# HKUST-Aerial-Robotics/ESVO

Hardware: AMD Instinct MI355X
Metric: mapped events/sec (stereo TS raster + block matching + LM depth refinement + fusion), events resident in HBM before the timed region; exactly K ticks between two synchronisations, i.e. including the fill and the drain of the two-deep tick pipeline (`sustained`: the same workload over 1600 ticks) (higher is better)
Workload: dtype f64

## Files before the change

esvo_amd/csrc/api_core.hip:

```cpp
#include "context.hpp"

namespace esvo_host {
thread_local std::string g_create_error;
}

namespace {

void invert3x3(const double* P, double* Kinv, double* Kinv_t) {
  const double a = P[0], b = P[1], cc = P[2], d = P[4], e = P[5], f = P[6], g = P[8], hh = P[9], i = P[10];
  const double det = a * (e * i - f * hh) - b * (d * i - f * g) + cc * (d * hh - e * g);
  const double id = 1.0 / det;
  Kinv[0] = (e * i - f * hh) * id; Kinv[1] = (cc * hh - b * i) * id; Kinv[2] = (b * f - cc * e) * id;
  Kinv[3] = (f * g - d * i) * id;  Kinv[4] = (a * i - cc * g) * id;  Kinv[5] = (cc * d - a * f) * id;
  Kinv[6] = (d * hh - e * g) * id; Kinv[7] = (b * g - a * hh) * id;  Kinv[8] = (a * e - b * d) * id;
  for (int r = 0; r < 3; ++r) Kinv_t[r] = (Kinv[r * 3 + 0] * P[3] + Kinv[r * 3 + 1] * P[7]) + Kinv[r * 3 + 2] * P[11];
}

int validate_params(const esvo_params_t* p, std::string& why) {
  if (p->ls_norm != ESVO_LSNORM_TDIST && p->ls_norm != ESVO_LSNORM_L2) { why = "LSnorm must be Tdist or l2 (DepthProblemSolver.cpp:121-131 exits on anything else)"; return ESVO_ERR_UNSUPPORTED; }
  if (p->bm_step < 1) { why = "BM_step must be >= 1"; return ESVO_ERR_INVALID_ARG; }
  if (p->patch_size_x < 1 || p->patch_size_x > 64 || p->patch_size_y < 1 || p->patch_size_y > 40) { why = "patch size must be within 1..64 x 1..40"; return ESVO_ERR_UNSUPPORTED; }
  if (p->median_blur_kernel_size < 0 || p->median_blur_kernel_size > 3) { why = "median_blur_kernel_size must be 0..3 (kernel 2k + 1)"; return ESVO_ERR_UNSUPPORTED; }
  if (p->max_event_queue_len < 0 || p->max_event_queue_len > TSQ_LMAX) { why = "max_event_queue_len must be 0 (one stamp per pixel) or 1..32"; return ESVO_ERR_UNSUPPORTED; }
  if (p->bm_max_disparity < p->bm_min_disparity || p->bm_min_disparity < 0) { why = "bad disparity range"; return ESVO_ERR_INVALID_ARG; }
// ... 133 lines not shown
  CK(h->d_tick_ev.alloc(E));
  CK(h->d_match_slots.alloc(E));
  CK(h->d_match_flags.alloc(E)); CK(h->d_match_prefix.alloc(E));
  for (int k = 0; k < 2; ++k) CK(h->front[k].d_matches.alloc(E));
  if (E >= LM_SPLIT_MIN_EVENTS) {
    CK(h->d_lm_fvec0.alloc(E * 7 * 16)); CK(h->d_lm_fnorm0.alloc(E));
    CK(h->d_lm_meta.alloc(E)); CK(h->d_lm_order.alloc(E));
    CK(h->d_lm_hist.alloc(2 * 32 * 64));
    CK(hipMemset(h->d_lm_hist, 0, sizeof(u32) * 2 * 32 * 64));
  }
  if (E > LM_TWO_QUEUES_MAX_EVENTS) {
    for (int k = 0; k < 2; ++k) { CK(h->front[k].d_lm_pix_order.alloc(E)); CK(h->d_lm_sort_rows[k].alloc(E)); }
    CK(h->d_lm_sort_hist.alloc(voxel_hist_words(E)));
  }
  if (h->bm_dedupe_on && E >= h->bm_dedupe_min) CK(h->d_bm_dedupe.alloc(npx + 4 + 2 * E));
  CK(h->d_clk.alloc(2 * clk_words(h->max_ev)));
  CK(hipMemset(h->d_clk, 0, sizeof(u64) * 2 * clk_words(h->max_ev)));
  int khz = 0;
  if (hipDeviceGetAttribute(&khz, hipDeviceAttributeWallClockRate, h->device) != hipSuccess || khz <= 0) khz = 100000;
  h->stats.clk_ref_khz = (uint32_t)khz;
  for (int k = 0; k < 2; ++k) {
    CK(h->front[k].d_pt_slots.alloc(E));
    CK(h->front[k].d_pt_flags.alloc(E)); CK(h->front[k].d_pt_prefix.alloc(E));
    CK(h->front[k].d_scan_tmp_l.alloc(scan_scratch_elems(std::max(E, npx)) + 8));
  }
  CK(h->d_pts_tmp.alloc(E));
  for (int k = 0; k < 2; ++k) CK(h->front[k].d_stage.alloc(E));
  for (int k = 0; k < 2; ++k) CK(h->front[k].d_counters.alloc(CNT_ROW));
  for (int k = 0; k < 2; ++k) CK(hipMemset(h->front[k].d_counters, 0, sizeof(u32) * CNT_ROW));
  CK(h->h_counters.alloc(CNT_ROW * 2));
  std::memset(h->h_counters, 0, sizeof(u32) * CNT_ROW * 2);
  CK(h->h_pin.alloc(2 * ((size_t)h->max_poses * 17 + 16)));
  CK(h->d_scan_tmp.alloc(scan_scratch_elems(std::max(E, npx)) + 8)); CK(h->d_scan_tmp_b.alloc(scan_scratch_elems(std::max(E, npx)) + 8));
  CK(h->d_cnt_b.alloc(CNTB_ROW)); CK(hipMemset(h->d_cnt_b, 0, sizeof(u32) * CNTB_ROW));
  CK(h->h_cnt_b.alloc(CNTB_ROW * CNTB_ROWS));
  std::memset(h->h_cnt_b, 0, sizeof(u32) * CNTB_ROW * CNTB_ROWS);
  for (int k = 0; k < 2; ++k) { h->front[k].d_clk = h->d_clk + (size_t)k * clk_words(h->max_ev); h->front[k].h_counters = h->h_counters + CNT_ROW * k; h->back[k].h_cnt = h->h_cnt_b + CNTB_ROW * k; }
  CK(h->d_halo_viol.alloc(2));
  return ESVO_OK;
}

int alloc_window_and_map(esvo_context* h) {
  const size_t npx = (size_t)h->W * h->H, E = h->max_ev;
  h->win_cap = (u32)std::max<int64_t>((int64_t)h->prm.max_window_points, (int64_t)E) + 2 * (u32)E;
  CK(h->d_win.alloc(h->win_cap));
  h->max_frames = (u32)std::max(h->prm.max_fusion_frames + 2, 512);
  if (h->prm.fusion_strategy == ESVO_FUSION_CONST_POINTS)
    h->max_frames = std::max(h->max_frames, (u32)(1.5 * h->prm.max_fusion_points) + 4u);
  h->slot_used.assign(h->max_frames + 1, 0);
  h->n_pose_slots = std::min<u32>(h->max_frames + 1, h->n_pose_slots);
  CK(h->d_frame_pose_T.alloc((size_t)h->n_pose_slots * h->max_poses * 16));
  CK(h->d_fr_table.alloc(2 * (3 * (size_t)h->max_frames + 1))); CK(h->h_fr_table.alloc(2 * (3 * (size_t)h->max_frames + 1)));
  for (int k = 0; k < 2; ++k) { h->back[k].d_fr_table = h->d_fr_table + k * (h->d_fr_table.cap() / 2); h->back[k].h_fr_table = h->h_fr_table + k * (h->h_fr_table.cap() / 2); }
  CK(h->d_prop.alloc(h->win_cap));
  const size_t n_tiles = fuse_front_tiles(h);
  CK(h->d_tile_pts.alloc(n_tiles * h->fuse_tile_cap)); CK(h->d_over_pts.alloc(h->win_cap));
  CK(h->d_tile_count.alloc(n_tiles));
  CK(h->d_cell_count.alloc(npx)); CK(h->d_cell_offset.alloc(npx));
  h->fuse_slice_cap = (u32)((n_tiles + 63) / 64) * FUSE_TILE * FUSE_TILE;
  CK(h->d_cell_list.alloc((size_t)16 * 64 * h->fuse_slice_cap));
  CK(h->d_fuse_ctr.alloc(2112 + 64));
  CK(hipMemset(h->d_fuse_ctr + 2112, 0, sizeof(u32) * 64));
  CK(h->d_rec_ids.alloc(n_tiles * h->fuse_tile_rec + (size_t)h->win_cap * 9));
  for (int k = 0; k < 2; ++k) CK(h->d_map_mem[k].alloc(map_buffer_bytes(npx)));
  h->d_map = reinterpret_cast<MapCell*>(h->d_map_mem[0].get()); h->d_map2 = reinterpret_cast<MapCell*>(h->d_map_mem[1].get());
  CK(h->d_owner_max.alloc(npx)); CK(h->d_owner_min.alloc(npx));
  CK(h->d_own_w.alloc(E)); CK(h->d_lkeep.alloc(E));
  h->codes_bytes = (E + 7) / 8 * 8;
  CK(h->d_codes.alloc(h->codes_bytes));
  CK(h->d_sel.alloc(E));
  CK(h->d_evmap.alloc(npx + 64));
  CK(h->d_reg_ab.alloc(npx)); CK(h->d_reg_cd.alloc(npx));
  CK(h->d_exp_flags.alloc(npx)); CK(h->d_exp_prefix.alloc(npx));
  CK(h->d_export.alloc(npx)); CK(h->d_export_cell.alloc(npx));
  return ESVO_OK;
}

int create_events_and_pools(esvo_context* h) {
  for (int k = 0; k < 2; ++k) CK(h->ts_ev[k].create());
  CK(h->ev_frame.create());
  for (int k = 0; k < 2; ++k) CK(h->front[k].own_ev.create());
  for (int k = 0; k < 2; ++k) { CK(h->back[k].ev.create()); CK(h->pose[k].released.create()); }
  if (h->tl_on) { CK(h->tl_ref.create()); CK(hipEventRecord(h->tl_ref, h->stream)); CK(hipEventSynchronize(h->tl_ref)); }
  CK(h->evt_trk_read.create(hipEventDisableTiming));
  for (int cam = 0; cam < 2; ++cam) CK(h->evt_ingest[cam].create(hipEventDisableTiming));
  CK(h->h_pose_pool.alloc(16 * (size_t)h->max_poses * esvo_context::POSE_POOL));
  for (int i = 0; i < esvo_context::POSE_POOL; ++i) CK(h->pool_evt[i].create());
  for (int i = 0; i < 16; ++i) h->T_world_obs[i] = h->T_world_frame[i] = (i % 5 == 0) ? 1.0 : 0.0;
  return ESVO_OK;
}
#undef CK

}

namespace esvo_host {

void fill_dev_params(esvo_context* h) {
  const esvo_params_t& p = h->prm;
  DevParams& d = h->dp;
  d.W = h->W; d.H = h->H;
  d.wx = p.patch_size_x; d.wy = p.patch_size_y;
  d.dmin = p.bm_min_disparity; d.dmax = p.bm_max_disparity; d.step = p.bm_step; d.updown = p.bm_updown ? 1 : 0;
  d.zncc_thr = p.bm_zncc_threshold;
  d.baseline_f = h->baseline * d.camL.P[0];
  d.td_nu = p.td_nu; d.td_scale = p.td_scale; d.td_scale2 = p.td_scale * p.td_scale;
  const double td_stdvar = std::sqrt(p.td_nu / (p.td_nu - 2) * (p.td_scale * p.td_scale));
  d.td_stdvar2 = td_stdvar * td_stdvar;
// ... 302 lines not shown
```

esvo_amd/csrc/api_window.hip:

```cpp
#include "context.hpp"

namespace esvo_host {

static int read_counters_b(esvo_context* h, int row, bool sync) {
  HIPCHK(hipMemcpyAsync(h->h_cnt_b + CNTB_ROW * row, h->d_cnt_b, sizeof(u32) * CNTB_ROW, hipMemcpyDeviceToHost, h->stream_b));
  if (sync) HIPCHK(hipStreamSynchronize(h->stream_b));
  return ESVO_OK;
}
int back_after_front(esvo_context* h) {
  HIPCHK(hipEventRecord(h->ev_frame, h->stream));
  HIPCHK(hipStreamWaitEvent(h->stream_b, h->ev_frame, 0));
  return ESVO_OK;
}
void collect_back(esvo_context* h, int par) {
  if (!h->back_pending[par]) return;
  h->back_pending[par] = false;
  const BackSlot& B = h->back[par];
  esvo_stats_t& s = h->stats;
  s.last_fusions = B.h_cnt[CNTB_FUSIONS];
  if (h->routed && h->h_cnt_b[CNTB_ROW * CNTB_ROW_HALO + par]) {
    s.halo_violations = h->h_cnt_b[CNTB_ROW * CNTB_ROW_HALO + par];
    h->halo_error = true;
  }
  if (h->prm.regularization) s.last_map_size = B.h_cnt[CNTB_REG_ELEMS];
// ... 126 lines not shown
      HIPCHK(hipEventRecord(h->pool_evt[ps], h->stream_b));
    } else if (h->pro.active) {
      h->pro.b_src = h->pose[pose_buf].d_T; h->pro.b_dst = dst; h->pro.b_bytes = sizeof(double) * 16 * m;
      h->pro.ev_b = h->pose[pose_buf].released;
    } else {
      HIPCHK(hipMemcpyAsync(dst, h->pose[pose_buf].d_T, sizeof(double) * 16 * m, hipMemcpyDeviceToDevice, h->stream_b));
      HIPCHK(hipEventRecord(h->pose[pose_buf].released, h->stream_b));
    }
  }
  h->frames.push_back(FrameRec{off, count, slot, 1});
  h->n_window_frames++;
  if (apply_policy) apply_window_policy(h);
  return ESVO_OK;
}

int run_fuse(esvo_context* h, int par, const double* T_world_obs, bool naive) {
  BackSlot& B = h->back[par];
  u32* host = B.h_fr_table;
  u32 nf = 0;
  for (size_t q = h->frames.size(); q-- > 0;)
    if (h->frames[q].count) ++nf;
  if (nf > h->max_frames) { (void)flush_deferred_copies(h); FAIL(ESVO_ERR_CAPACITY, "too many non-empty frames in the fusion window"); }
  u32* cum = host;
  u32* off = host + (nf + 1);
  u32* slot = off + nf;
  u32 total = 0, i = 0;
  for (size_t q = h->frames.size(); q-- > 0;) {
    const FrameRec& f = h->frames[q];
    if (f.count == 0) continue;
    cum[i] = total; off[i] = f.off; slot[i] = f.slot;
    total += f.count;
    ++i;
  }
  cum[nf] = total;
  hipStream_t sb = h->stream_b;
  hipEvent_t tail_ev[2] = {nullptr, nullptr};
  u32* dtab = B.d_fr_table;
  if (h->pro.active) {
    const esvo_context::DeferredCopies d = h->pro;
    h->pro = esvo_context::DeferredCopies();
    launch_back_prologue(host, dtab, sizeof(u32) * (3 * (size_t)nf + 1), d.a_src, d.a_dst, d.a_bytes, d.b_src, d.b_dst, d.b_bytes, sb,
                         d.a_flags, d.a_prefix, d.a_slots);
    tail_ev[0] = d.ev_a; tail_ev[1] = d.ev_b;
  } else {
    launch_upload_words(host, dtab, sizeof(u32) * (3 * (size_t)nf + 1), sb);
  }
  std::memcpy(h->T_world_frame, T_world_obs, sizeof(double) * 16);
  FuseArgs a;
  a.win = h->d_win;
  a.fr_cum = dtab; a.fr_off = dtab + (nf + 1); a.fr_slot = a.fr_off + nf;
  a.n_frames = nf; a.n_pts = total;
  a.frame_pose_T = h->d_frame_pose_T; a.max_poses = h->max_poses;
  rigid_inverse(h->T_world_frame, a.T_frame_world);
  a.prop = h->d_prop;
  a.tile_count = h->d_tile_count; a.tile_pts = h->d_tile_pts; a.tile_cap = h->fuse_tile_cap;
  a.over_pts = h->d_over_pts; a.over_count = h->d_fuse_ctr + FUSE_CTR_OVER_COUNT;
  a.rec_ids = h->d_rec_ids; a.tile_rec = h->fuse_tile_rec; a.rec_cursor = h->d_fuse_ctr + FUSE_CTR_REC_CURSOR;
  a.cell_count = h->d_cell_count; a.cell_offset = h->d_cell_offset; a.cell_list = h->d_cell_list; a.slice_cap = h->fuse_slice_cap;
  a.class_count = h->d_fuse_ctr; a.class_total = h->d_fuse_ctr + FUSE_CTR_CLASS_TOTAL;
  a.lds_cap = h->fuse_lds_cap; a.pmax_plus1 = h->fuse_pmax_plus1; a.d_total = h->d_cnt_b + CNTB_RECORDS;
  a.map = h->d_map; a.d_num_fusion = h->d_cnt_b + CNTB_FUSIONS;
  a.n_touched = h->d_cnt_b + CNTB_TOUCHED;
  a.naive = naive ? 1 : 0;
  a.owner_max = h->prm.regularization ? h->d_owner_max : nullptr;
  a.owner_min = h->d_owner_min; a.n_reg_elems = h->prm.regularization ? h->d_cnt_b + CNTB_REG_ELEMS : nullptr;
  if (total > h->win_cap) {
    for (hipEvent_t e : tail_ev) if (e) hipEventRecord(e, sb);
    FAIL(ESVO_ERR_CAPACITY, "window points exceed capacity");
  }
  const bool timed = h->stage_events_on;
  B.timed = timed;
  if (timed) hipEventRecord(B.ev.e[BE_FU0], sb);
  launch_fuse(a, h->dp, sb);
  if (timed) hipEventRecord(B.ev.e[BE_FU1], sb);
  h->d_map_cur = h->d_map;
  h->map_id_bound = total * ((naive || h->dp.fusion_radius == 0) ? 4u : 9u);
  const bool do_clean = naive ? false : (h->prm.clean_requires_full_window ? (h->n_window_frames >= (size_t)h->prm.max_fusion_frames) : true);
  if (do_clean) launch_clean(h->d_map, h->dp, sb);
  if (timed) hipEventRecord(B.ev.e[BE_CL1], sb);
  if (h->prm.regularization && !naive) {
    launch_reg_view(h->d_map, h->d_map2, h->d_owner_max, h->d_owner_min, h->d_reg_ab, h->d_reg_cd, h->d_cnt_b + CNTB_REG_ELEMS, h->dp, sb);
    const u64 band_cells = (u64)std::max(h->dp.band_y1 - h->dp.band_y0, 1) * (u64)h->W;
    const bool sparse = h->reg_sparse_forced >= 0 ? h->reg_sparse_forced == 1 : (u64)h->stats.last_map_size * 10u < band_cells;
    launch_reg_apply(h->d_map, h->d_map2, h->d_owner_max, h->d_owner_min, h->d_reg_ab, h->d_reg_cd, h->d_cnt_b + CNTB_REG_ELEMS, h->dp, sb, sparse);
    h->d_map_cur = h->d_map2;
  }
  HIPCHK(hipMemcpyAsync(B.h_cnt, h->d_cnt_b, sizeof(u32) * CNTB_ROW, hipMemcpyDeviceToHost, sb));
  if (h->routed) HIPCHK(hipMemcpyAsync(h->h_cnt_b + CNTB_ROW * CNTB_ROW_HALO + par, h->d_halo_viol, sizeof(u32), hipMemcpyDeviceToHost, sb));
  hipEventRecord(B.ev.e[BE_RG1], sb);
  for (hipEvent_t e : tail_ev) if (e) hipEventRecord(e, sb);
  HIPCHK(hipGetLastError());
  h->back_pending[par] = true;
  return ESVO_OK;
}

int export_map(esvo_context* h, std::vector<esvo_depth_point_t>& out, std::vector<u32>* cells) {
  launch_map_compact(h->d_map_cur, h->d_exp_flags, h->d_exp_prefix, h->d_cnt_b + CNTB_MAP, h->d_scan_tmp_b, h->d_export,
                     h->d_export_cell, h->dp, h->stream_b);
  int rc = read_counters_b(h, CNTB_ROW_EXPORT, true);
  if (rc) return rc;
  const u32 n = h->h_cnt_b[CNTB_ROW * CNTB_ROW_EXPORT + CNTB_MAP];
  out.resize(n);
  std::vector<u32> cell(n);
  if (n) {
    HIPCHK(hipMemcpy(out.data(), h->d_export, sizeof(esvo_depth_point_t) * n, hipMemcpyDeviceToHost));
    HIPCHK(hipMemcpy(cell.data(), h->d_export_cell, sizeof(u32) * n, hipMemcpyDeviceToHost));
  }
// ... 132 lines not shown
```

esvo_amd/csrc/common.hpp:

```cpp
#pragma once

#include <hip/hip_runtime.h>
#include <stdint.h>

#include "../../include/esvo_hip.h"

#define ESVO_WAVE 64

#include <cstdlib>
#include <cstring>
inline const char* esvo_dev_switch(const char* name) {
  const char* on = std::getenv("ESVO_DEV_SWITCHES");
  return (on && std::strcmp(on, "1") == 0) ? std::getenv(name) : nullptr;
}

namespace esvo {

typedef unsigned long long u64;
typedef unsigned int u32;

struct CamConst {
  double P[12];
  double Kinv[9];
  double Kinv_t[3];
// ... 319 lines not shown
void launch_shard_codes_routed(const esvo_match_t* own_matches, const u32* keep, const u32* n_local, u32 max_local, u32 n, u32 T, u32* own_w,
                               u32* block, hipStream_t s);
void launch_shard_unpack_routed(const u32* blocks, u32 block_words, u32 N, u32 n, uint8_t* codes, u32* rank_kept, u32* tile_sums, hipStream_t s);

bool lm_launch_is_wide(u32 max_matches, const struct DevParams& p);
struct LmArgs {
  const esvo_match_t* matches;
  const u32* n_matches;
  u32 max_matches;
  const uint8_t* tsL;
  const uint8_t* tsR;
  const double* pose_T;
  double T_world_obs[16];
  DevPoint* out_slots;
  u32* out_flags;
  int cull;
  int dense;
  double* split_fvec0;
  double* split_fnorm0;
  u32* split_meta;
  u32* split_order;
  u32* split_hist;
  int pair;
  const u32* match_index;
  const u32* order = nullptr;
  u64* clk;
  u32* halo_viol = nullptr;
  int vy0 = 0, vy1 = 0;
};
constexpr u32 LM_GUARD_STRIPES = 32, LM_GUARD_WORDS = 8;
struct LmGuard {
  u32* stripes = nullptr;
  int limit = 0;
};
void launch_lm_guard_fold(u32* stripes, u32* counter_row, hipStream_t s);
constexpr u32 CLK_XCDS = 8, CLK_SAMPLES = 16, CLK_SCRATCH = 32, CLK_STRIDE = 65;
inline size_t clk_words(u32 max_ev) { return CLK_SCRATCH + 2 * ((size_t)max_ev / 64 + 2); }
constexpr u32 LM_PAIR_MAX_EVENTS = 10000u;
constexpr u32 LM_TWO_QUEUES_MAX_EVENTS = 40000u;
#ifndef LM_SPLIT_MIN
#define LM_SPLIT_MIN 400000u
#endif
constexpr u32 LM_SPLIT_MIN_EVENTS = LM_SPLIT_MIN;
void launch_lm_refine(const LmArgs& a, const DevParams& p, u32* n_solved, hipStream_t s, const LmGuard& g = LmGuard());
bool lm_launch_is_ordered(u32 max_matches, bool dense, bool band, bool split, const DevParams& p);
int lm_order_variant();
u32 lm_order_key(u32 x, u32 y, u32 ssd, int W, int H);
void launch_lm_pixel_order(const esvo_match_t* matches, const u32* n_matches, u32 max_matches, int dense, const uint8_t* tsL,
                           const uint8_t* tsR, const DevParams& p, u64* const rows[2], u32* hist, u32* scan_tmp, u32* order, hipStream_t s);
void launch_compact_points(const DevPoint* slots, const u32* flags, const u32* prefix, const u32* n_in,
                           u32 max_n, DevPoint* out, hipStream_t s);

#define FUSE_TILE 8
struct FuseArgs {
  const DevPoint* win;
  const u32* fr_cum;
  const u32* fr_off;
  const u32* fr_slot;
  u32 n_frames;
  u32 n_pts;
  const double* frame_pose_T;
  u32 max_poses;
  double T_frame_world[16];
  DevPoint* prop;
  u32* tile_count;
  uint2* tile_pts;
  u32 tile_cap;
  uint2* over_pts;
  u32* over_count;
  u32* rec_ids;
  u32 tile_rec;
  u32* rec_cursor;
  u32* cell_count;
  u32* cell_offset;
  u32* cell_list;
  u32 slice_cap;
  u32* class_count;
  u32* class_total;
  u32 lds_cap;
  u32 pmax_plus1;
  u32* d_total;
  MapCell* map;
  u32* d_num_fusion;
  u32* n_touched;
  int naive;
  u32* owner_max;
  u32* owner_min;
  u32* n_reg_elems;
};
void launch_fuse(const FuseArgs& a, const DevParams& p, hipStream_t s);
void launch_clean(MapCell* map, const DevParams& p, hipStream_t s);
void launch_reg_view(const MapCell* map_in, MapCell* map_out, u32* owner_max, u32* owner_min, double2* ab, double2* cd,
                     u32* n_elems, const DevParams& p, hipStream_t s);
void launch_reg_apply(const MapCell* map_in, MapCell* map_out, const u32* owner_max, const u32* owner_min, const double2* ab,
                      const double2* cd, u32* n_elems, const DevParams& p, hipStream_t s, bool sparse = false);
struct SgmScratch {
  uint8_t *sobL, *rawL, *sobR, *rawR;
  int16_t* vol[6];
  int16_t *d1, *d1b;
  u32* d2key;
};
void launch_sgbm(const uint8_t* left, const uint8_t* right, const SgmScratch& s, int16_t* disp, int W, int H, hipStream_t st);
void launch_sgm_points(const esvo_event_t* ring, u64 first, u64 cap, u32 n, const float2* lut, const int16_t* disp, DevPoint* slots,
                       u32* flags, const DevParams& p, hipStream_t st);
void launch_sgm_tick_points(const esvo_event_t* ev, u64 first, u64 cap, int reverse, u32 n, const float2* lut, const int16_t* disp,
                            DevPoint* slots, u32* flags, u32* cnt, const DevParams& p, hipStream_t st);
void launch_sgm_naive(const DevPoint* pts, u32 n, const double* d_T_frame_obs, u32* owner, u32* pair_flags, u32* pair_rank, u32* d_total,
                      u32* scan_tmp, MapCell* map, const DevParams& p, hipStream_t st);
void launch_debug_image(const MapCell* map, u32* owner, uint8_t* bgr, const uint8_t* jet, int type, double max_range,
                        double min_range, double thr1, double thr2, const DevParams& p, hipStream_t s);
void launch_map_compact(const MapCell* map, u32* flags, u32* prefix, u32* d_total, u32* scan_tmp,
                        esvo_depth_point_t* out, u32* out_cell, const DevParams& p, hipStream_t s);
void launch_map_cloud(const MapCell* map, u32 id_n, u32* present, u32* prefix, u32* where, u32* counts, u32* scan_tmp, const double* T_world_frame,
                      float* xyz, u32 cap_points, const DevParams& p, hipStream_t s);

void launch_map_cloud_near(const MapCell* map, u32 id_n, double range, u32* present, u32* prefix, u32* where, u32* counts, u32* scan_tmp,
                           const double* T_world_frame, float* xyz, u32 cap_points, const DevParams& p, hipStream_t s);
// ... 20 lines not shown
```

esvo_amd/csrc/context.hpp:

```cpp
#pragma once
#include <algorithm>
#include <array>
#include <atomic>
#include <chrono>
#include <cmath>
#include <cstdio>
#include <cstdlib>
#include <cstring>
#include <deque>
#include <mutex>
#include <string>
#include <vector>

#include "common.hpp"
#include "devmem.hpp"
#include "ring_spans.hpp"

using namespace esvo;

struct FrameRec {
  u32 off;
  u32 count;
  u32 slot;
  u32 run;
// ... 168 lines not shown
  std::vector<u32> hist_free;
  DevEvent evt_hist;
  DevBuf<esvo_event_t> d_ring[2];
  DevBuf<uint8_t> d_wire[2];
  DevBuf<uint8_t> d_col[2];
  PinBuf<u64> h_col_stamps[2];
  size_t col_cap[2] = {0, 0};
  DevBuf<uint16_t> d_evt3_words[2];
  DevBuf<u32> d_evt3_tiles[2], d_evt3_hdr[2];
  PinBuf<u32> h_evt3_hdr[2];
  size_t evt3_device_min = 24576;
  u64 ring_cap = 0;
  DevEvent evt_ingest[2];

  DevBuf<uint8_t> d_obs_tmp;

  PoseBuf pose[2];
  int pose_buf = 0;
  std::vector<double> h_pose_T;
  PinBuf<double> h_pin;

  u32 max_ev = 0;
  DevBuf<esvo_event_t> d_tick_ev;
  DevBuf<esvo_match_t> d_match_slots;
  DevBuf<u32> d_match_flags, d_match_prefix;
  DevBuf<double> d_lm_fvec0, d_lm_fnorm0;
  DevBuf<u32> d_lm_meta, d_lm_order, d_lm_hist;
  DevBuf<u64> d_lm_sort_rows[2];
  DevBuf<u32> d_lm_sort_hist;
  bool lm_order_on = true;
  DevBuf<u32> d_bm_dedupe;
  bool bm_dedupe_on = true;
  u32 bm_dedupe_min = esvo::BM_DEDUPE_MIN_EVENTS;
  DevBuf<u64> d_clk;
  bool clk_probe = true;
  DevBuf<DevPoint> d_pts_tmp;
  PinBuf<u32> h_counters;
  DevBuf<u32> d_scan_tmp;
  DevBuf<u32> d_cnt_b;
  PinBuf<u32> h_cnt_b;
  DevBuf<u32> d_scan_tmp_b;

  DevBuf<DevPoint> d_win;
  u32 win_cap = 0;
  u32 n_pose_slots = 0;
  std::vector<char> slot_used;
  DevBuf<double> d_frame_pose_T;
  u32 max_poses = 0;
  DevBuf<u32> d_fr_table;
  PinBuf<u32> h_fr_table;
  u32 max_frames = 0;

  DevBuf<DevPoint> d_prop;
  DevBuf<u32> d_tile_count;
  DevBuf<uint2> d_tile_pts, d_over_pts;
  DevBuf<u32> d_cell_count, d_cell_offset, d_cell_list;
  DevBuf<u32> d_fuse_ctr;
  u32 fuse_tile_rec = 4096;
  u32 fuse_slice_cap = 0;
  u32 fuse_tile_cap = 1024;
  u32 fuse_pmax_plus1 = 0;
  DevBuf<u32> d_rec_ids;
  u32 fuse_lds_cap = 0;
  DevBuf<uint8_t> d_map_mem[2];
  DevBuf<u32> d_owner_max, d_owner_min;
  DevBuf<u32> d_sel;
  DevBuf<uint8_t> d_evmap;
  DevBuf<u32> d_own_w;
  DevBuf<u32> d_lkeep;
  DevBuf<uint8_t> d_codes;
  size_t codes_bytes = 0;
  DevBuf<uint8_t> d_codes_send;
  DevBuf<uint8_t> d_codes_all;
  DevBuf<unsigned long long> d_pts_send;
  DevBuf<unsigned long long> d_pts_all;
  DevBuf<u32> d_rank_kept;
  static constexpr u32 SHARD_MAX_RANKS = 1024;
  bool sharded = false;
  bool routed = false;
  int ts_halo = 0;
  int rband_y0 = 0, rband_y1 = 0;
  int oband_y0 = 0, oband_y1 = 0;
  int sband_y0[2] = {0, 0}, sband_y1[2] = {0, 0};
  std::vector<int> fix_row_lo[2], fix_row_hi[2];
  std::vector<uint8_t> keep_px;
  DevBuf<u32> d_ring_gidx;
  PinBuf<esvo_event_t> h_route_ev[2];
  PinBuf<u32> h_route_gidx;
  size_t route_cap[2] = {0, 0};
  DevBuf<esvo_event_t> d_merge_a, d_merge_b;
  DevBuf<u32> d_merge_plan;
  DevBuf<esvo_event_t> d_tsq_dup;
  DevBuf<u32> d_halo_viol;
  DevBuf<u32> d_dn_flags;
  int lm_pair_forced = -1;
  FrontSlot front[2];
  int fpar = 0;
  FrontSlot& front_cur() { return front[fpar]; }
  bool tick_pending = false;
  BackSlot back[2];
  TsEvents ts_ev[2];
  DevEvent ev_frame;
  int tsq_len = 0;
  DevBuf<u64> d_tsq[2];
  DevBuf<u32> d_tsq_tcount;
  DevBuf<uint4> d_tsq_tlist, d_tsq_over;
// ... 181 lines not shown
```

esvo_amd/csrc/kernels_fuse.hip:

```cpp
#include <algorithm>
#include <type_traits>
#define DEV_HOOKS_FUSE_TU
#include "common.hpp"
#include "dev_hooks.hpp"
#include "fdiv.hpp"
#include "scan.hpp"

namespace esvo {

#ifndef BACK_WAVES
#define BACK_WAVES 6
#endif
#ifndef FUSE_WAVES
#define FUSE_WAVES 1
#endif

__device__ inline bool boundaryCheck(double x, double y, int W, int H) {
  return !(x < 0 || x >= (double)W || y < 0 || y >= (double)H);
}

__device__ inline bool fusion_cell(u32 prow, u32 pcol, int k, int radius, int W, int H, int& row, int& col) {
  int dy, dx;
  if (radius == 0) { dy = k >> 1; dx = k & 1; }
  else { dy = k / 3 - 1; dx = k % 3 - 1; }
// ... 24 lines not shown
  if (q >= a.n_pts) return;
  u32 f = 0;
  {
    u32 lo = 0, hi = a.n_frames;
    while (hi - lo > 1) { const u32 mid = (lo + hi) >> 1; if (a.fr_cum[mid] <= q) lo = mid; else hi = mid; }
    f = lo;
  }
  const DevPoint prior = a.win[a.fr_off[f] + (q - a.fr_cum[f])];
  const double* pose = a.frame_pose_T + ((size_t)a.fr_slot[f] * a.max_poses + prior.pose_idx) * 16;
  double T[16];
  mat4_mul(a.T_frame_world, pose, T);
  DevPoint prop;
  double pp[3];
#pragma unroll
  for (int r = 0; r < 3; ++r)
    pp[r] = ((T[r * 4 + 0] * prior.p_cam[0] + T[r * 4 + 1] * prior.p_cam[1]) + T[r * 4 + 2] * prior.p_cam[2]) + T[r * 4 + 3];
  double u, v;
  world2Cam(p.camL, pp, u, v);
  if (!boundaryCheck(u, v, p.W, p.H) || !(u == u) || !(v == v)) {
    prop.row = 0xffffffffu;
    prop.col = 0;
    a.prop[q] = prop;
    return;
  }
  prop.row = (u32)(size_t)floor(v);
  prop.col = (u32)(size_t)floor(u);
  prop.x[0] = u;
  prop.x[1] = v;
  const double invDepth = 1.0 / pp[2];
  double denominator = (T[8] * prior.p_cam[0] + T[9] * prior.p_cam[1]) + T[11];
  denominator /= prior.p_cam[2];
  denominator += T[10];
  const double J = T[10] / (denominator * denominator);
  prop.inv_depth = invDepth;
  if constexpr (MODEL == FUSE_TDIST) {
    const double scale2 = J * J * prior.scale2;
    const double nu = prior.nu;
    prop.scale2 = scale2;
    prop.variance = nu / (nu - 2) * scale2;
    prop.nu = nu;
  } else {
    double variance = J * J * prior.variance;
    if (variance < 1e-6) variance = 1e-6;
    prop.variance = variance;
    prop.scale2 = 0;
    prop.nu = 0;
  }
  prop.p_cam[0] = pp[0]; prop.p_cam[1] = pp[1]; prop.p_cam[2] = pp[2];
  prop.residual = prior.residual;
  prop.age = prior.age;
  prop.pose_idx = 0;
  prop.seq = q;
  a.prop[q] = prop;
  (void)K;
  const u32 tile = (prop.row / FT) * (u32)fuse_tiles_x(p.W) + prop.col / FT;
  const uint2 entry = make_uint2(q, (prop.row << 16) | prop.col);
  const u32 pos = atomicAdd(&a.tile_count[tile], 1u);
  if (pos < a.tile_cap) a.tile_pts[(size_t)tile * a.tile_cap + pos] = entry;
  else a.over_pts[atomicAdd(a.over_count, 1u)] = entry;
}

__device__ inline void update_studentT(MapCell& c, double invD, double s2, double var, double nu_in) {
  if (c.inv_depth > -1e-6) {
    const double nu_update = (c.nu < nu_in) ? c.nu : nu_in;
    const Recip rsum = make_recip(c.scale2 + s2);
    const double n1 = s2 * c.inv_depth + c.scale2 * invD;
    const double dd = c.inv_depth - invD;
    const double n2 = dd * dd;
    const double invDepth_update = div_by(n1, rsum);
    const double scale2_update = div_by((nu_update + div_by(n2, rsum)) / (nu_update + 1) * (c.scale2 * s2), rsum);
    c.inv_depth = invDepth_update;
    c.scale2 = scale2_update;
    c.nu = nu_update + 1;
    c.variance = c.nu / (c.nu - 2) * c.scale2;
    c.age++;
  } else {
    c.inv_depth = invD; c.scale2 = s2; c.variance = var; c.nu = nu_in;
  }
}

template <int MODEL>
__device__ inline void fuse_record(const DevParams& p, MapCell& c, bool& exists, u32& numFusion, const DevPoint& prop, u32 id, int crow,
                                   int ccol) {
  if (!exists) {
    c.row = (u32)crow; c.col = (u32)ccol;
    c.x[0] = (double)ccol + 0.5; c.x[1] = (double)crow + 0.5;
    c.inv_depth = prop.inv_depth; c.scale2 = prop.scale2; c.variance = prop.variance; c.nu = prop.nu;
    if (MODEL != FUSE_TDIST && c.variance < 1e-6) c.variance = 1e-6;
    c.residual = prop.residual;
    c.age = prop.age;
    cam2World(p.camL, c.x[0], c.x[1], prop.inv_depth, c.p_cam);
    c.seq = id;
    exists = true;
    return;
  }
  if constexpr (MODEL == FUSE_NAIVE) {
    if (c.inv_depth > prop.inv_depth) return;
    if (prop.residual < c.residual) {
      c.row = prop.row; c.col = prop.col;
      c.x[0] = prop.x[0]; c.x[1] = prop.x[1];
      c.inv_depth = prop.inv_depth; c.scale2 = prop.scale2; c.nu = prop.nu; c.variance = prop.variance;
      c.residual = prop.residual; c.age = prop.age;
      c.p_cam[0] = prop.p_cam[0]; c.p_cam[1] = prop.p_cam[1]; c.p_cam[2] = prop.p_cam[2];
    }
    return;
  } else {
    bool compatible;
    if constexpr (MODEL == FUSE_L2) {
      const double d = prop.inv_depth - c.inv_depth, dd = d * d;
      compatible = dd / prop.variance + dd / c.variance < 5.99;
    } else {
      const double s1 = sqrt(prop.variance), s2 = sqrt(c.variance), diff = fabs(prop.inv_depth - c.inv_depth);
      compatible = diff < 2 * s1 || diff < 2 * s2;
    }
    if (compatible) {
      if constexpr (MODEL == FUSE_L2) {
        if (c.inv_depth > -1e-6) {
          const double temp = c.inv_depth, tv = c.variance;
          c.inv_depth = (tv * prop.inv_depth + prop.variance * temp) / (tv + prop.variance);
          c.variance = (tv * prop.variance) / (tv + prop.variance);
        } else {
          c.inv_depth = prop.inv_depth;
          c.variance = prop.variance;
        }
        if (c.variance < 1e-6) c.variance = 1e-6;
      } else {
        update_studentT(c, prop.inv_depth, prop.scale2, prop.variance, prop.nu);
      }
      c.age++;
      c.residual = (prop.residual < c.residual) ? prop.residual : c.residual;
      cam2World(p.camL, c.x[0], c.x[1], prop.inv_depth, c.p_cam);
      numFusion++;
    } else {
      if (c.inv_depth - 2 * sqrt(c.variance) > prop.inv_depth) return;
      if (prop.variance < c.variance && prop.residual < c.residual) {
        c.row = prop.row; c.col = prop.col;
        c.x[0] = prop.x[0]; c.x[1] = prop.x[1];
        c.inv_depth = prop.inv_depth; c.scale2 = prop.scale2; c.nu = prop.nu; c.variance = prop.variance;
        c.residual = prop.residual; c.age = prop.age;
        c.p_cam[0] = prop.p_cam[0]; c.p_cam[1] = prop.p_cam[1]; c.p_cam[2] = prop.p_cam[2];
      }
    }
  }
}

#define FUSE_PMAX 1024
#define FUSE_BITW (FUSE_PMAX / 32 + 1)
#define FUSE_BUF (FUSE_LDS_CAP_MAX > 2 * FUSE_PMAX + FT_CELLS * FUSE_BITW ? FUSE_LDS_CAP_MAX : 2 * FUSE_PMAX + FT_CELLS * FUSE_BITW)
__global__ void __launch_bounds__(FT_CELLS, 8) tile_lists_kernel(FuseArgs a, DevParams p, int K, int radius, u32 cap, u32 pmax) {
  __shared__ u32 s_buf[FUSE_BUF];
  __shared__ u32 s_cnt[FT_CELLS];
  __shared__ u32 s_off[FT_CELLS + 1];
  __shared__ u32 s_fill[FT_CELLS];
  __shared__ u32 s_tmp[FUSE_SORT_TMP];
  __shared__ u32 s_scan[1];
  __shared__ u32 s_hist[FUSE_NB], s_hbase[FUSE_NB];
  const int lane = threadIdx.x;
  const int tiles_x = fuse_tiles_x(p.W), tiles_y = fuse_tiles_y(p.H);
  const int tx = (int)(blockIdx.x % tiles_x), ty = (int)(blockIdx.x / tiles_x);
  const int r0 = ty * FT, c0 = tx * FT;
  const int crow = r0 + lane / FT, ccol = c0 + lane % FT;
  const int ncell = p.W * p.H;
  const bool in_img = crow < p.H && ccol < p.W;
  const bool in_band = in_img && crow >= p.cband_y0 && crow < p.cband_y1;
  const int cell = crow * p.W + ccol;
  const u64 lt_mask = (1ull << lane) - 1ull;
  if (lane < FUSE_NB) s_hist[lane] = 0;
  if (in_img && a.owner_max) { a.owner_max[cell] = 0; a.owner_min[cell] = 0xffffffffu; }
  const int f_lo = radius == 0 ? 0 : -1, f_hi = 1;
  auto reaches = [&](u32 prow, u32 pcol) {
    return (int)prow + f_hi >= r0 && (int)prow + f_lo < r0 + FT && (int)pcol + f_hi >= c0 && (int)pcol + f_lo < c0 + FT;
  };
  const u32 n_over = *a.over_count;
  auto for_lists = [&](auto&& fn) {
    for (int dy = -1; dy <= 1; ++dy) {
      const int ny = ty + dy;
      if (ny < 0 || ny >= tiles_y) continue;
      for (int dx = -1; dx <= 1; ++dx) {
        const int nx = tx + dx;
        if (nx < 0 || nx >= tiles_x) continue;
        const int nt = ny * tiles_x + nx;
        u32 cnt = a.tile_count[nt];
        if (cnt > a.tile_cap) cnt = a.tile_cap;
        fn(a.tile_pts + (size_t)nt * a.tile_cap, cnt);
      }
    }
    fn(a.over_pts, n_over);
  };
  u32* s_q = s_buf;
  u32* s_rc = s_buf + FUSE_PMAX;
  u32 P = 0;
  const uint2* lptr[10];
  u32 lpref[11];
  {
// ... 214 lines not shown
      }
      u64 longm = __ballot(mine && n > 24);
      while (longm) {
        const int src = __ffsll((long long)longm) - 1;
        longm &= longm - 1;
        const u32 ln = (u32)__shfl((int)n, src), lo = (u32)__shfl((int)(s_off[lane] - base), src);
        u32* lid = s_ids + lo;
        if (ln <= FUSE_SORT_TMP) {
          for (u32 i = (u32)lane; i < ln; i += ESVO_WAVE) {
            const u32 vkey = lid[i];
            u32 rk = 0;
            for (u32 j = 0; j < ln; ++j) rk += (lid[j] < vkey);
            s_tmp[rk] = vkey;
          }
          __builtin_amdgcn_wave_barrier();
          for (u32 i = (u32)lane; i < ln; i += ESVO_WAVE) lid[i] = s_tmp[i];
          __builtin_amdgcn_wave_barrier();
        } else if (lane == src) {
          for (u32 i = 1; i < ln; ++i) {
            const u32 key = lid[i];
            int j = (int)i - 1;
            while (j >= 0 && lid[j] > key) { lid[j + 1] = lid[j]; --j; }
            lid[j + 1] = key;
          }
        }
      }
      __syncthreads();
      for (u32 i = (u32)lane; i < run_n; i += ESVO_WAVE) gout[base + i] = s_ids[i];
      __syncthreads();
    } else {
      u32* gids = gout + base;
      expand([&](int lc, u32 id) {
        if ((u32)lc == run0) gids[atomicAdd(&s_fill[lc], 1u)] = id;
      });
      __threadfence_block();
      __syncthreads();
      if (mine) {
        for (u32 i = 1; i < n; ++i) {
          const u32 key = gids[i];
          long long j = (long long)i - 1;
          while (j >= 0 && gids[j] > key) { gids[j + 1] = gids[j]; --j; }
          gids[j + 1] = key;
        }
      }
      __syncthreads();
    }
    run0 = run1;
  }
}

#ifndef FUSE_BLOCK
#define FUSE_BLOCK 256
#endif
template <int MODEL>
__global__ void __launch_bounds__(FUSE_BLOCK, FUSE_WAVES) fuse_cells_kernel(FuseArgs a, DevParams p, int K, int n_tiles) {
  const u32 t = blockIdx.x * blockDim.x + threadIdx.x;
  const int ncell = p.W * p.H;
  constexpr u32 NSEG = FUSE_NB * FUSE_SLICES;
  __shared__ u32 s_seg[NSEG + 1];
  for (u32 i = threadIdx.x; i <= NSEG; i += FUSE_BLOCK) s_seg[i] = a.class_total[i];
  __syncthreads();
  if (t >= s_seg[NSEG]) return;
  u32 lo = 0, hi = NSEG;
  while (hi - lo > 1) { const u32 mid = (lo + hi) >> 1; if (s_seg[mid] <= t) lo = mid; else hi = mid; }
  const u32 cls = FUSE_NB - 1u - lo / FUSE_SLICES, slc = lo % FUSE_SLICES;
  const int cell = (int)a.cell_list[((size_t)cls * FUSE_SLICES + slc) * a.slice_cap + (t - s_seg[lo])];
  const int crow = cell / p.W, ccol = cell - crow * p.W;
  const u32 n = a.cell_count[cell];
  const u32* ids = a.rec_ids + a.cell_offset[cell];
  MapCell c;
  bool exists = false;
  u32 numFusion = 0;
  u32 id_nxt = ids[0];
  DevPoint nxt = a.prop[id_nxt / (u32)K];
  for (u32 i = 0; i < n; ++i) {
    const u32 id = id_nxt;
    const DevPoint prop = nxt;
    if (i + 1 < n) {
      id_nxt = ids[i + 1];
      nxt = a.prop[id_nxt / (u32)K];
    }
    fuse_record<MODEL>(p, c, exists, numFusion, prop, id, crow, ccol);
  }
  a.map[cell] = c;
  map_flags(a.map, ncell)[cell] = CELL_ALIVE | CELL_GRID;
  if (numFusion) atomicAdd(a.d_num_fusion, numFusion);
  (void)n_tiles;
}

#define FUSE_TURN_B 256
__global__ void __launch_bounds__(FUSE_TURN_B) fuse_turn_kernel(FuseArgs a, int n_tiles) {
  __shared__ u32 lds[FUSE_TURN_B / ESVO_WAVE];
  constexpr u32 NSEG = FUSE_NB * FUSE_SLICES;
  constexpr u32 PER = NSEG / FUSE_TURN_B;
  static_assert(NSEG % FUSE_TURN_B == 0, "segments per thread");
  u32 c[PER], sum = 0;
#pragma unroll
  for (u32 k = 0; k < PER; ++k) {
    const u32 seg = threadIdx.x * PER + k;
    const u32 cls = FUSE_NB - 1u - seg / FUSE_SLICES, slc = seg % FUSE_SLICES;
    c[k] = a.class_count[cls * FUSE_SLICES + slc];
    a.class_count[cls * FUSE_SLICES + slc] = 0;
    sum += c[k];
  }
  u32 tot;
  u32 ex = block_excl_scan<FUSE_TURN_B / ESVO_WAVE>(sum, &tot, lds);
#pragma unroll
  for (u32 k = 0; k < PER; ++k) { a.class_total[threadIdx.x * PER + k] = ex; ex += c[k]; }
  for (int i = (int)threadIdx.x; i < n_tiles; i += FUSE_TURN_B) a.tile_count[i] = 0;
  if (threadIdx.x == 0) {
    a.class_total[NSEG] = tot;
    *a.n_touched = tot;
    *a.d_total = *a.rec_cursor;
    *a.rec_cursor = 0;
    *a.over_count = 0;
    *a.d_num_fusion = 0;
    if (a.n_reg_elems) *a.n_reg_elems = 0;
  }
}

void launch_fuse(const FuseArgs& a, const DevParams& p, hipStream_t s) {
  const int ncell = p.W * p.H;
  const int model = a.naive ? FUSE_NAIVE : (p.ls_norm == ESVO_LSNORM_L2 ? FUSE_L2 : FUSE_TDIST);
  const int K = (model == FUSE_NAIVE || p.fusion_radius == 0) ? 4 : 9;
  const int radius = model == FUSE_NAIVE ? 0 : p.fusion_radius;
  const int n_tiles = fuse_tiles_x(p.W) * fuse_tiles_y(p.H);
  if (a.n_pts) {
    const dim3 g((a.n_pts + 255) / 256), b(256);
    if (model == FUSE_TDIST) hipLaunchKernelGGL(propagate_kernel<FUSE_TDIST>, g, b, 0, s, a, p, K);
    else if (model == FUSE_L2) hipLaunchKernelGGL(propagate_kernel<FUSE_L2>, g, b, 0, s, a, p, K);
    else hipLaunchKernelGGL(propagate_kernel<FUSE_NAIVE>, g, b, 0, s, a, p, K);
  }
  const u32 cap = (a.lds_cap >= 1 && a.lds_cap <= FUSE_LDS_CAP_MAX) ? a.lds_cap : FUSE_LDS_CAP_MAX;
  const u32 pmax = a.pmax_plus1 ? std::min<u32>(a.pmax_plus1 - 1u, FUSE_PMAX) : FUSE_PMAX;
  hipLaunchKernelGGL(tile_lists_kernel, dim3(n_tiles), dim3(FT_CELLS), 0, s, a, p, K, radius, cap, pmax);
  hipLaunchKernelGGL(fuse_turn_kernel, dim3(1), dim3(FUSE_TURN_B), 0, s, a, n_tiles);
// ... 393 lines not shown
```

Baseline: 188.5 million.

## Split fusion operands into compact struct and defer cam2World to cell end

The propagation kernel now also writes a compact 48-byte FuseOperand per point (inv_depth, scale2, nu, variance, residual, precomputed sqrt of variance). The fuse-cells loop prefetches only these compact operands, two ids ahead, instead of a full DevPoint. It reads the full point only when a replacement happens, and it does a single cam2World per cell at the end instead of one per fused record. It also replaces the integer divide by K with a shift or a constant divide. The cost is an extra write stream and an extra buffer in the propagation kernel, and more state to keep correct, such as the pending flag semantics on replacement.

```diff
diff --git a/esvo_amd/csrc/api_core.hip b/esvo_amd/csrc/api_core.hip
--- a/esvo_amd/csrc/api_core.hip
+++ b/esvo_amd/csrc/api_core.hip
@@ -209,7 +209,7 @@
   CK(h->d_frame_pose_T.alloc((size_t)h->n_pose_slots * h->max_poses * 16));
   CK(h->d_fr_table.alloc(2 * (3 * (size_t)h->max_frames + 1))); CK(h->h_fr_table.alloc(2 * (3 * (size_t)h->max_frames + 1)));
   for (int k = 0; k < 2; ++k) { h->back[k].d_fr_table = h->d_fr_table + k * (h->d_fr_table.cap() / 2); h->back[k].h_fr_table = h->h_fr_table + k * (h->h_fr_table.cap() / 2); }
-  CK(h->d_prop.alloc(h->win_cap));
+  CK(h->d_prop.alloc(h->win_cap)); CK(h->d_prop_ops.alloc(h->win_cap));
   const size_t n_tiles = fuse_front_tiles(h);
   CK(h->d_tile_pts.alloc(n_tiles * h->fuse_tile_cap)); CK(h->d_over_pts.alloc(h->win_cap));
   CK(h->d_tile_count.alloc(n_tiles));
diff --git a/esvo_amd/csrc/api_window.hip b/esvo_amd/csrc/api_window.hip
--- a/esvo_amd/csrc/api_window.hip
+++ b/esvo_amd/csrc/api_window.hip
@@ -202,7 +202,7 @@
   a.n_frames = nf; a.n_pts = total;
   a.frame_pose_T = h->d_frame_pose_T; a.max_poses = h->max_poses;
   rigid_inverse(h->T_world_frame, a.T_frame_world);
-  a.prop = h->d_prop;
+  a.prop = h->d_prop; a.ops = h->d_prop_ops;
   a.tile_count = h->d_tile_count; a.tile_pts = h->d_tile_pts; a.tile_cap = h->fuse_tile_cap;
   a.over_pts = h->d_over_pts; a.over_count = h->d_fuse_ctr + FUSE_CTR_OVER_COUNT;
   a.rec_ids = h->d_rec_ids; a.tile_rec = h->fuse_tile_rec; a.rec_cursor = h->d_fuse_ctr + FUSE_CTR_REC_CURSOR;
diff --git a/esvo_amd/csrc/common.hpp b/esvo_amd/csrc/common.hpp
--- a/esvo_amd/csrc/common.hpp
+++ b/esvo_amd/csrc/common.hpp
@@ -395,6 +395,11 @@
                            u32 max_n, DevPoint* out, hipStream_t s);
 
 #define FUSE_TILE 8
+struct alignas(16) FuseOperand {
+  double inv_depth, scale2, nu, variance, residual;
+  double sd;
+};
+static_assert(sizeof(FuseOperand) == 48, "FuseOperand layout");
 struct FuseArgs {
   const DevPoint* win;
   const u32* fr_cum;
@@ -406,6 +411,7 @@
   u32 max_poses;
   double T_frame_world[16];
   DevPoint* prop;
+  FuseOperand* ops;
   u32* tile_count;
   uint2* tile_pts;
   u32 tile_cap;
diff --git a/esvo_amd/csrc/context.hpp b/esvo_amd/csrc/context.hpp
--- a/esvo_amd/csrc/context.hpp
+++ b/esvo_amd/csrc/context.hpp
@@ -244,6 +244,7 @@
   u32 max_frames = 0;
 
   DevBuf<DevPoint> d_prop;
+  DevBuf<FuseOperand> d_prop_ops;
   DevBuf<u32> d_tile_count;
   DevBuf<uint2> d_tile_pts, d_over_pts;
   DevBuf<u32> d_cell_count, d_cell_offset, d_cell_list;
diff --git a/esvo_amd/csrc/kernels_fuse.hip b/esvo_amd/csrc/kernels_fuse.hip
--- a/esvo_amd/csrc/kernels_fuse.hip
+++ b/esvo_amd/csrc/kernels_fuse.hip
@@ -100,6 +100,14 @@
   prop.pose_idx = 0;
   prop.seq = q;
   a.prop[q] = prop;
+  {
+    FuseOperand op;
+    op.inv_depth = prop.inv_depth; op.scale2 = prop.scale2; op.nu = prop.nu; op.variance = prop.variance;
+    op.residual = prop.residual;
+    if constexpr (MODEL == FUSE_TDIST) op.sd = sqrt(prop.variance);
+    else op.sd = 0;
+    a.ops[q] = op;
+  }
   (void)K;
   const u32 tile = (prop.row / FT) * (u32)fuse_tiles_x(p.W) + prop.col / FT;
   const uint2 entry = make_uint2(q, (prop.row << 16) | prop.col);
@@ -127,30 +135,33 @@
   }
 }
 
+__device__ inline void replace_cell(MapCell& c, bool& pending, const FuseOperand& prop, const DevPoint* pt) {
+  c.row = pt->row; c.col = pt->col;
+  c.x[0] = pt->x[0]; c.x[1] = pt->x[1];
+  c.inv_depth = prop.inv_depth; c.scale2 = prop.scale2; c.nu = prop.nu; c.variance = prop.variance;
+  c.residual = prop.residual; c.age = pt->age;
+  c.p_cam[0] = pt->p_cam[0]; c.p_cam[1] = pt->p_cam[1]; c.p_cam[2] = pt->p_cam[2];
+  pending = false;
+}
+
 template <int MODEL>
-__device__ inline void fuse_record(const DevParams& p, MapCell& c, bool& exists, u32& numFusion, const DevPoint& prop, u32 id, int crow,
-                                   int ccol) {
+__device__ inline void fuse_record(MapCell& c, bool& exists, u32& numFusion, bool& pending, double& pending_inv, const FuseOperand& prop,
+                                   const DevPoint* pt, u32 id, int crow, int ccol) {
   if (!exists) {
     c.row = (u32)crow; c.col = (u32)ccol;
     c.x[0] = (double)ccol + 0.5; c.x[1] = (double)crow + 0.5;
     c.inv_depth = prop.inv_depth; c.scale2 = prop.scale2; c.variance = prop.variance; c.nu = prop.nu;
     if (MODEL != FUSE_TDIST && c.variance < 1e-6) c.variance = 1e-6;
     c.residual = prop.residual;
-    c.age = prop.age;
-    cam2World(p.camL, c.x[0], c.x[1], prop.inv_depth, c.p_cam);
+    c.age = pt->age;
+    pending = true; pending_inv = prop.inv_depth;
     c.seq = id;
     exists = true;
     return;
   }
   if constexpr (MODEL == FUSE_NAIVE) {
     if (c.inv_depth > prop.inv_depth) return;
-    if (prop.residual < c.residual) {
-      c.row = prop.row; c.col = prop.col;
-      c.x[0] = prop.x[0]; c.x[1] = prop.x[1];
-      c.inv_depth = prop.inv_depth; c.scale2 = prop.scale2; c.nu = prop.nu; c.variance = prop.variance;
-      c.residual = prop.residual; c.age = prop.age;
-      c.p_cam[0] = prop.p_cam[0]; c.p_cam[1] = prop.p_cam[1]; c.p_cam[2] = prop.p_cam[2];
-    }
+    if (prop.residual < c.residual) replace_cell(c, pending, prop, pt);
     return;
   } else {
     bool compatible;
@@ -158,7 +169,7 @@
       const double d = prop.inv_depth - c.inv_depth, dd = d * d;
       compatible = dd / prop.variance + dd / c.variance < 5.99;
     } else {
-      const double s1 = sqrt(prop.variance), s2 = sqrt(c.variance), diff = fabs(prop.inv_depth - c.inv_depth);
+      const double s1 = prop.sd, s2 = sqrt(c.variance), diff = fabs(prop.inv_depth - c.inv_depth);
       compatible = diff < 2 * s1 || diff < 2 * s2;
     }
     if (compatible) {
@@ -177,17 +188,11 @@
       }
       c.age++;
       c.residual = (prop.residual < c.residual) ? prop.residual : c.residual;
-      cam2World(p.camL, c.x[0], c.x[1], prop.inv_depth, c.p_cam);
+      pending = true; pending_inv = prop.inv_depth;
       numFusion++;
     } else {
       if (c.inv_depth - 2 * sqrt(c.variance) > prop.inv_depth) return;
-      if (prop.variance < c.variance && prop.residual < c.residual) {
-        c.row = prop.row; c.col = prop.col;
-        c.x[0] = prop.x[0]; c.x[1] = prop.x[1];
-        c.inv_depth = prop.inv_depth; c.scale2 = prop.scale2; c.nu = prop.nu; c.variance = prop.variance;
-        c.residual = prop.residual; c.age = prop.age;
-        c.p_cam[0] = prop.p_cam[0]; c.p_cam[1] = prop.p_cam[1]; c.p_cam[2] = prop.p_cam[2];
-      }
+      if (prop.variance < c.variance && prop.residual < c.residual) replace_cell(c, pending, prop, pt);
     }
   }
 }
@@ -508,6 +513,7 @@
 #ifndef FUSE_BLOCK
 #define FUSE_BLOCK 256
 #endif
+__device__ inline u32 fuse_point_of(u32 id, int K) { return K == 4 ? id >> 2 : id / 9u; }
 template <int MODEL>
 __global__ void __launch_bounds__(FUSE_BLOCK, FUSE_WAVES) fuse_cells_kernel(FuseArgs a, DevParams p, int K, int n_tiles) {
   const u32 t = blockIdx.x * blockDim.x + threadIdx.x;
@@ -527,17 +533,24 @@
   MapCell c;
   bool exists = false;
   u32 numFusion = 0;
+  bool pending = false;
+  double pending_inv = 0;
   u32 id_nxt = ids[0];
-  DevPoint nxt = a.prop[id_nxt / (u32)K];
+  u32 id_nxt2 = n > 1 ? ids[1] : 0u;
+  u32 q_nxt = fuse_point_of(id_nxt, K);
+  FuseOperand nxt = a.ops[q_nxt];
   for (u32 i = 0; i < n; ++i) {
-    const u32 id = id_nxt;
-    const DevPoint prop = nxt;
+    const u32 id = id_nxt, q = q_nxt;
+    const FuseOperand prop = nxt;
     if (i + 1 < n) {
-      id_nxt = ids[i + 1];
-      nxt = a.prop[id_nxt / (u32)K];
-    }
-    fuse_record<MODEL>(p, c, exists, numFusion, prop, id, crow, ccol);
-  }
+      id_nxt = id_nxt2;
+      q_nxt = fuse_point_of(id_nxt, K);
+      nxt = a.ops[q_nxt];
+      if (i + 2 < n) id_nxt2 = ids[i + 2];
+    }
+    fuse_record<MODEL>(c, exists, numFusion, pending, pending_inv, prop, a.prop + q, id, crow, ccol);
+  }
+  if (pending) cam2World(p.camL, c.x[0], c.x[1], pending_inv, c.p_cam);
   a.map[cell] = c;
   map_flags(a.map, ncell)[cell] = CELL_ALIVE | CELL_GRID;
   if (numFusion) atomicAdd(a.d_num_fusion, numFusion);
```

After: 188.5 million. About the same (-0.0%).
